# teshnizi/GraphEnvs

Hardware: AMD Instinct MI355X
Metric: env-steps/sec (whole node), ShortestPath-v0 n=64 m=192 batch=65536, 1/2/4/8 GPU (higher is better)
Workload: dtype u64; 1 GPU; ShortestPath-v0 n_nodes=64 n_edges=192 weighted, 65536 env slots per GPU, random valid actions on device, same-step autoreset (seed-exact G(n,m)+features on device); envs_per_gpu=65536, prefetch_period=0, episodes_finished_per_gpu=6165512, settle_steps=128, parallelism=batch shard x1, no collective

## Files before the change

graphenvs_amd/csrc/ge_api.hip:

```cpp
#include <math.h>
#include <stdio.h>
#include <stdlib.h>
#include <string.h>

#include <initializer_list>
#include <memory>
#include <new>
#include <vector>

#include "ge_params.h"
#include "ge_platform.h"
#include "ge_reset.h"
#include "ge_features.h"
#include "ge_step.h"
#include "ge_tsp_eval.h"
#include "ge_spare.h"
#include "ge_policy.h"

#define GE_MAX_BUCKETS 4
struct GeBucket {
  bool used;
  bool list_only;
  struct { int lds, pre, grid; } graph;
  struct { int lds, pre_off, threads, grid; } gen;
};
struct GePlan {
  int n_buckets;
  GeBucket bk[GE_MAX_BUCKETS];
  int nseed;
  int nseed2;
  bool feat_fast;
  int f64_lds, f64_pre_off, feat_grid;
  GeLds inject;
  int pol_group, pol_grid;
};
static int bucket_of(int n) { return n <= 128 ? 0 : (n <= 256 ? 1 : (n <= 512 ? 2 : 3)); }
static bool takes_generic(const GeParams &C) { return C.n > 64 || C.spatial; }

typedef void (*GeBaselineFn)(GeParams, GeRagged, int, uint8_t *, uint64_t);
struct GeKernels {
  void (*reset)(GeParams, GeRagged, const uint32_t *, GeRun, GeInject, int, int);
  void (*features)(GeParams, GeRagged, GeRun, int, int);
  void (*features64)(GeParams, GeRagged, GeRun, int);
  void (*feat_combine)(GeParams, GeRagged, GeRun);
  void (*swap)(GeParams, GeRagged, GeRagged, ge_buffers, int);
  void (*sample)(GeParams, GeRagged, uint64_t, int64_t *);
  void (*policy_head[GE_POL_MODES])(GeParams, GeRagged, GePolicyIO);
  void (*policy_grad)(GeParams, GeRagged, GePolicyIO);
  void (*dc_range)(GeParams, GeRagged, const int64_t *);
  void (*tsp_closure)(GeParams, GeRagged, int, uint8_t *, uint64_t, int);
  GeBaselineFn tsp_tour, mis_baseline, steiner_baseline;
  void (*step[2])(GeParams, GeRagged, const int64_t *, uint64_t);
  int step_threads;
  size_t step_lds;
  bool step_quad;
  void (*step_path64[2][2])(GeParams, const int64_t *, uint64_t);
};

struct ge_engine {
  GeParams P;
  ge_config cfg;
  GeKernels k = {};
  GePlan plan = {};
  hipEvent_t ev[4];
  bool have_events = false;
  int n_classes = 0;
  GeRagged R = {};
  int aw_max;
  std::vector<GeParams> classes;
  bool loaded = false;
  bool seeded = false;
  bool streams = false;
  bool spares = false;
  GeParams PS;
  GeRagged RS = {};
  std::vector<GeParams> classesS;
  int period = 0, swap_parts = 1;
  int64_t pending_calls = 0;
  int32_t *refill_list = nullptr, *refill_count = nullptr;
};

static GeRun run_full() { GeRun r = {GE_ITEMS_ALL, 1, 0, 0, 0, 0, 0}; return r; }
static GeRun run_inject(bool seeds) { GeRun r = {GE_ITEMS_ALL, seeds ? 2 : 0, 0, 0, 1, 0, 0}; return r; }
static GeRun run_continue() { GeRun r = {GE_ITEMS_ALL, 0, 1, 1, 0, 0, 0}; return r; }
static GeRun run_queue(const ge_engine *e) { GeRun r = {GE_ITEMS_QUEUE, 0, 1, 0, 0, 0, e->spares ? 2 : GE_SEED_DEPTH, e->plan.nseed2}; return r; }
static GeRun run_refill() { GeRun r = {GE_ITEMS_QUEUE, 0, 1, 0, 0, 1, 2}; return r; }
static GeRun as_list(GeRun r) { r.items = GE_ITEMS_LIST; return r; }


static thread_local char g_err[256] = "";
static int fail(int code, const char *msg) { snprintf(g_err, sizeof(g_err), "%s", msg); return code; }
extern "C" const char *ge_last_error(void) { return g_err; }
extern "C" int ge_abi_version(void) { return GE_ABI_VERSION; }
#ifndef GE_SOURCE_HASH
#define GE_SOURCE_HASH "unknown"
#endif
static const char g_source_hash[] = "GE_SOURCE_HASH=" GE_SOURCE_HASH;
extern "C" const char *ge_source_hash(void) { return g_source_hash + 15; }

static const int kMaxLds = 160 * 1024;
static const GeInject kNoInject = {nullptr, nullptr, nullptr, nullptr, nullptr};
static int step_blocks(int64_t B) { return (int)((B + GE_STEP_BLOCK - 1) / GE_STEP_BLOCK); }
static int prefix_bytes(int64_t B) { return (step_blocks(B) + 2) * 4; }
static bool carves_fit(std::initializer_list<int> bytes) { for (int b : bytes) if (b > kMaxLds) return false; return true; }
static int resident_grid(int lds, int64_t B) {
  int per_cu = kMaxLds / (lds > 0 ? lds : 1);
  if (per_cu > 16) per_cu = 16;
  if (per_cu < 1) per_cu = 1;
// ... 128 lines not shown
  if (P.feat_parts > 1 && !bufs->feat_scratch) return fail(GE_E_BADARG, "feat_scratch required (ge_layout.feat_parts > 1)");
  if (P.spatial && !bufs->sw64) return fail(GE_E_BADARG, "spatial TSP needs sw64");
  if (eval_slot_bytes(P) && !bufs->eval_scratch) return fail(GE_E_BADARG, "is_eval_env of TSP / unweighted MaxIndependentSet / SteinerTree (1 < n_dests < n - 1) needs eval_scratch (ge_layout.eval_scratch_bytes)");
  if (P.W == 1 && !bufs->node_rec) return fail(GE_E_BADARG, "n_nodes <= 64 needs node_rec");
  if (prunes(P) && P.W > GE_MAXW && !bufs->prune_scratch)
    return fail(GE_E_BADARG, "parenting >= 2 on more than 512 nodes needs prune_scratch ([B, 4, W] uint64)");
  return GE_OK;
}

static bool edge_quad(const ge_engine *e) {
  static const bool off = getenv("GE_NO_EDGE_QUAD") != nullptr;
  return !off && (e->P.env_type == GE_STEINER_TREE || e->P.env_type == GE_MULTICAST_ROUTING) && ge_edge_fits(e->aw_max, e->P.W);
}

static bool path64(const ge_engine *e) {
  return e->n_classes == 0 && (e->P.env_type == GE_SHORTEST_PATH || e->P.env_type == GE_LONGEST_PATH) && e->P.W == 1 && e->P.parenting < 2;
}

template <int ENV, bool RAGGED>
static void select_kernels(ge_engine *e) {
  GeKernels &k = e->k;
  k.reset = ge_k_reset<ENV, RAGGED>;
  k.features = ge_k_features<RAGGED>;
  k.features64 = ge_k_features64<RAGGED>;
  k.feat_combine = ge_k_feat_combine<RAGGED>;
  k.swap = ge_k_swap<RAGGED>;
  k.sample = ge_k_sample<RAGGED>;
  k.policy_head[GE_POL_SAMPLE] = ge_k_policy_head<RAGGED, GE_POL_SAMPLE>;
  k.policy_head[GE_POL_GREEDY] = ge_k_policy_head<RAGGED, GE_POL_GREEDY>;
  k.policy_head[GE_POL_EVALUATE] = ge_k_policy_head<RAGGED, GE_POL_EVALUATE>;
  k.policy_grad = ge_k_policy_grad<RAGGED>;
  k.dc_range = ge_k_dc_range<RAGGED>;
  k.tsp_closure = ge_k_tsp_closure<RAGGED>;
  k.tsp_tour = ge_k_tsp_tour<RAGGED>;
  k.mis_baseline = ge_k_mis_baseline<RAGGED>;
  k.steiner_baseline = ge_k_steiner_baseline<RAGGED>;
  k.step[0] = ge_k_step<ENV, false, RAGGED, 0>; k.step[1] = ge_k_step<ENV, true, RAGGED, 0>;
  k.step_threads = GE_STEP_BLOCK;
  k.step_lds = (size_t)GE_STEP_BLOCK * e->P.W * 8 + GE_STEP_BLOCK + 64;
  if constexpr (ENV == GE_STEINER_TREE || ENV == GE_MULTICAST_ROUTING) {
    if (edge_quad(e)) {
      k.step[0] = ge_k_step_edge<ENV, false, RAGGED>; k.step[1] = ge_k_step_edge<ENV, true, RAGGED>;
      k.step_quad = true;
      k.step_threads = GE_EDGE_THREADS;
      k.step_lds = ge_edge_lds_bytes(e->aw_max, e->P.W) + (RAGGED ? GE_EDGE_CLASS_BYTES : 0);
    }
  }
// ... 42 lines not shown
    if (gen > gen_body) gen_body = gen;
    K.graph.grid = resident_grid(graph, P.B);
    K.graph.pre = P.lds.pre; K.graph.lds = graph;
    if (rg && P.lds.pre != 0) K.graph.lds = behind(graph, K.graph.pre);
    if (K.graph.lds > graph_lds) graph_lds = K.graph.lds;
    K.gen.threads = GE_WAVE * waves;
    K.gen.pre_off = P.ldsf.pre; K.gen.lds = P.ldsf.total;
    if (rg) K.gen.lds = behind(K.list_only ? all : gen, K.gen.pre_off);
    K.gen.grid = resident_grid(K.gen.lds, P.B);
    if (K.list_only && (rg || K.gen.grid > 8)) K.gen.grid = 8;
    if (K.gen.lds > gen_lds) gen_lds = K.gen.lds;
  }
  if (!rg) L.inject = inject_carve(P, P.B);
  if (!carves_fit({graph_lds, L.inject.total, gen_lds})) return fail(GE_E_TOOBIG, "per-env graph does not fit 160 KiB of LDS");
  L.nseed = (resident_grid(graph_lds, P.B) + 63) / 64;
  if (!raise_lds((const void *)e->k.reset, graph_lds > L.inject.total ? graph_lds : L.inject.total)) return fail(GE_E_LAUNCH, "cannot raise the dynamic LDS limit of the reset kernel");
  if (!raise_lds((const void *)e->k.step[0], e->k.step_lds) || !raise_lds((const void *)e->k.step[1], e->k.step_lds))
    return fail(GE_E_LAUNCH, e->k.step_quad ? "cannot raise the dynamic LDS limit of the edge step kernel" : "cannot raise the dynamic LDS limit of the step kernel");
  L.f64_pre_off = ge_align16(f64_body);
  L.f64_lds = L.feat_fast ? L.f64_pre_off + GE_F64_ITEMS * 4 * 4 + 16 : 0;
  L.nseed2 = (GE_SEED_SPLIT && !rg && L.feat_fast) ? (L.nseed * GE_WAVE + GE_SEED2_ITEMS - 1) / GE_SEED2_ITEMS : 0;
  const int seed2_lds = GE_SEED2_WAVES * GE_SEED2_WAVE_BYTES;
  if (L.nseed2 > 0 && L.f64_lds < seed2_lds) L.f64_lds = seed2_lds;
  if (!carves_fit({L.f64_lds})) return fail(GE_E_TOOBIG, "feature kernel does not fit LDS");
  if (!raise_lds((const void *)e->k.features, gen_lds)) return fail(GE_E_LAUNCH, "cannot raise the dynamic LDS limit of the feature kernel");
  if (L.feat_fast && !raise_lds((const void *)e->k.features64, L.f64_lds)) return fail(GE_E_LAUNCH, "cannot raise the dynamic LDS limit of the n<=64 feature kernel");
  L.feat_grid = resident_grid(L.feat_fast ? L.f64_lds : gen_body, P.B);
  int a_max = 0;
  for (const GeParams *C = first; C < first + n_classes; C++) if (C->A > a_max) a_max = C->A;
  L.pol_group = 4;
  while (L.pol_group < 64 && L.pol_group < a_max) L.pol_group <<= 1;
  const int64_t waves = ((int64_t)P.B * L.pol_group + GE_WAVE - 1) / GE_WAVE;
  L.pol_grid = (int)((waves + GE_POL_THREADS / GE_WAVE - 1) / (GE_POL_THREADS / GE_WAVE));
  return GE_OK;
}

extern "C" int ge_create(const ge_config *cfg, const ge_buffers *bufs, ge_engine **out) {
  if (!bufs || !out) return fail(GE_E_BADARG, "null argument");
  GeParams P;
  int rc = derive(cfg, P);
  if (rc != GE_OK) return rc;
  rc = check_buffers(P, bufs);
  if (rc != GE_OK) return rc;
  P.buf = *bufs;
  std::unique_ptr<ge_engine> e(new (std::nothrow) ge_engine());
  if (!e) return fail(GE_E_BADARG, "out of host memory");
  e->P = P; e->cfg = *cfg; e->aw_max = P.AW;
  rc = finish_create(e.get());
  if (rc == GE_OK) *out = e.release();
// ... 111 lines not shown
  int rc = GE_OK;
  if (e->n_classes == 0) rc = check_image(e->P, sp[0].image);
  for (int c = 0; c < e->n_classes && rc == GE_OK; c++) rc = check_image(e->classes[c], sp[c].image);
  if (rc != GE_OK) return rc;
  e->refill_list = sp[0].refill_list; e->refill_count = sp[0].refill_count;
  e->PS = image_view(e->P, sp[0].image, e->refill_list, e->refill_count);
  if (e->n_classes > 0) {
    e->classesS.resize(e->n_classes);
    for (int c = 0; c < e->n_classes; c++) e->classesS[c] = image_view(e->classes[c], sp[c].image, e->refill_list, e->refill_count);
    if (hipMemcpy(class_table_spare, e->classesS.data(), sizeof(GeParams) * (size_t)e->n_classes, hipMemcpyHostToDevice) != hipSuccess)
      return fail(GE_E_LAUNCH, "cannot copy the spare class table to the device");
    e->RS = e->R; e->RS.classes = (const GeParams *)class_table_spare;
  }
  e->P.spare_state = sp[0].state; e->P.swap_list = sp[0].swap_list; e->P.swap_count = sp[0].swap_count;
  e->PS.spare_state = sp[0].state;
  e->period = sp[0].period; e->pending_calls = 0;
  const GeParams &P = e->P;
  const int64_t slot_bytes = (int64_t)P.n * P.F * 4 + (int64_t)P.E * (16 + 4 * P.Fe + 2 + 1 + (P.buf.rev_edge ? 4 : 0)) + (int64_t)P.n * P.W * 8 * (P.buf.range_bits ? 2 : 1) + P.A;
  int parts = (int)(slot_bytes / 8192); if (parts < 1) parts = 1; if (parts > 16) parts = 16;
  if (parts >= 4) parts = GE_SWAP_GROUPS;
  e->swap_parts = parts;
  e->spares = true;
  e->plan.nseed2 = 0;
  return GE_OK;
}

extern "C" int ge_destroy(ge_engine *e) {
  if (!e) return GE_OK;
  if (e->have_events) for (int k = 0; k < 4; k++) (void)hipEventDestroy(e->ev[k]);
  delete e;
  return GE_OK;
}

static int check_launch(const char *what) {
  static const bool debug_sync = getenv("GE_DEBUG_SYNC") != nullptr;
  if (debug_sync) {
    fprintf(stderr, "[graphenvs] %s ...\n", what); fflush(stderr);
    const hipError_t hs = hipDeviceSynchronize();
    fprintf(stderr, "[graphenvs] %s %s\n", what, hs == hipSuccess ? "done" : hipGetErrorString(hs)); fflush(stderr);
    if (hs != hipSuccess) { snprintf(g_err, sizeof(g_err), "%s: %s (GE_DEBUG_SYNC)", what, hipGetErrorString(hs)); return GE_E_LAUNCH; }
  }
  hipError_t hr = hipGetLastError();
  if (hr != hipSuccess) { snprintf(g_err, sizeof(g_err), "%s: %s", what, hipGetErrorString(hr)); return GE_E_LAUNCH; }
  return GE_OK;
}

// ... 18 lines not shown
  const int g = spread(e->plan.feat_grid, B, queue);
  return small && g > 64 ? 64 : g;
}

static int generic_grid(const ge_engine *e, const GeBucket &K, const GeParams &V, GeRun run, bool small) {
  const bool queue = run.items == GE_ITEMS_QUEUE, list = e->plan.feat_fast;
  if (K.list_only) return K.gen.grid;
  int64_t want = list ? (int64_t)K.gen.grid * (queue ? 1 : 4) : fast_grid(e, V.B, queue, small);
  want *= ge_feat_workgroups(V.feat_parts);
  if (!list && queue && !run.refill && want > 4608) want = 4608;
  if (small && want > 288) want = 288;
  return want > 65535 * 16 ? 65535 * 16 : (int)want;
}

static int launch_features(ge_engine *e, const GeParams &V, const GeRagged &VR, GeRun run, bool small, void *stream) {
  const GePlan &L = e->plan;
  const GeRun rest = L.feat_fast ? as_list(run) : run;
  int rc = GE_OK;
  if (L.feat_fast) {
    const bool queue = run.items == GE_ITEMS_QUEUE;
    const int nseed2 = queue ? run.seed_split : 0;
    int grid = fast_grid(e, V.B, queue, small) - nseed2;
    if (grid < 1) grid = 1;
    GE_LAUNCH(e->k.features64, grid + nseed2, GE_F64_THREADS, L.f64_lds, stream, V, VR, run, L.f64_pre_off);
    rc = check_launch("feature kernel (n <= 64)");
  }
  for (int b = 0; b < L.n_buckets && rc == GE_OK; b++) {
    const GeBucket &K = L.bk[b];
    if (!K.used) continue;
    GE_LAUNCH(e->k.features, generic_grid(e, K, V, run, small), K.gen.threads, K.gen.lds, stream, V, VR, rest, K.gen.pre_off, e->n_classes > 0 ? b : -1);
    rc = check_launch(L.feat_fast ? "feature kernel (fallback list)" : "feature kernel");
  }
  if (rc != GE_OK || V.feat_parts == 1) return rc;
  return launch_combine(e, V, VR, rest, small, stream);
}

static int launch_seq_baseline(ge_engine *e, const GeParams &P, const GeRagged &VR, int queue, void *stream) {
  const uint64_t slot_bytes = e->n_classes > 0 ? 0 : eval_slot_bytes(P);
  const int pre = prefix_bytes(P.B);
  int g = (P.B + GE_TSP_EVAL_THREADS - 1) / GE_TSP_EVAL_THREADS; if (g > 4096) g = 4096;
  if (P.env_type == GE_MAX_INDEPENDENT_SET) {
    GE_LAUNCH(e->k.mis_baseline, g, GE_TSP_EVAL_THREADS, pre, stream, P, VR, queue, (uint8_t *)P.buf.eval_scratch, slot_bytes);
    return check_launch("MaxIndependentSet baseline kernel");
  }
  if (P.env_type == GE_STEINER_TREE) {
    GE_LAUNCH(e->k.steiner_baseline, g, GE_TSP_EVAL_THREADS, pre, stream, P, VR, queue, (uint8_t *)P.buf.eval_scratch, slot_bytes);
    return check_launch("SteinerTree baseline kernel");
// ... 351 lines not shown
```

graphenvs_amd/csrc/ge_features.h:

```cpp
#pragma once
#include "ge_params.h"
#include "ge_platform.h"
#include "ge_reset.h"

struct GeFctx {
  uint64_t *abits; int *rowptr; uint16_t *scw;
  uint64_t *quads; uint32_t *rq; int zq;
  uint8_t *c8;
  double *sigma, *delta, *coeff, *bcw;
  double *bcw0; int wave_f64;
  double *bc, *clos;
  double *prx, *prn, *sinv, *diff, *diff2, *clus;
  uint8_t *mark;
  uint16_t *ord, *lvl;
};

GE_DEV GeFctx ge_carve_f(const GeParams &P, int tid) {
  unsigned char *s = ge_dyn_smem();
  const GeLdsF &L = P.ldsf;
  const int n = P.n, an = ((n * 8 + 15) & ~15) / 8;
  GeFctx c;
  c.rowptr = (int *)(s + L.rowptr); c.quads = (uint64_t *)(s + L.colw); c.c8 = (uint8_t *)(s + L.colw); c.rq = (uint32_t *)(s + L.rq); c.zq = L.zq;
  c.bc = (double *)(s + L.bc); c.clos = (double *)(s + L.clos);
  unsigned char *w = s + L.wave0 + (tid >> 6) * L.wave_stride;
// ... 640 lines not shown
  for (int64_t g = (int64_t)ge_bid() * ge_bdim() + ge_tid(); g < (int64_t)count * nmax; g += (int64_t)ge_gdim() * ge_bdim()) {
    const int item = (int)(g / nmax), v = (int)(g % nmax);
    int env = queue ? ge_queue_slot(P, pre, item) : (list ? P.buf.work_list[item] : item);
    int cls = 0;
    if constexpr (RAGGED) { cls = R.slot_class[env]; env -= R.class_start[cls]; }
    const GeParams &C = RAGGED ? R.classes[cls] : P;
    const int n = C.n, nparts = C.feat_parts;
    if (v >= n || nparts == 1) continue;
    double acc = 0.0;
    for (int p = 0; p < nparts; p++) acc += C.buf.feat_scratch[((int64_t)env * nparts + p) * n + v];
    if (n > 2) acc *= 1.0 / (double)((int64_t)(n - 1) * (int64_t)(n - 2));
    C.buf.x[((int64_t)env * n + v) * C.F + C.nflag + 1] = (float)acc;
  }
}

#ifndef GE_F64_WPS
#define GE_F64_WPS 6
#endif
#if GE_F64_WPS > 0
#define GE_F64_KERNEL GE_KERNEL_LB(GE_F64_THREADS, GE_F64_WPS)
#else
#define GE_F64_KERNEL GE_KERNEL
#endif
template <bool RAGGED>
GE_F64_KERNEL ge_k_features64(GeParams P, GeRagged R, GeRun run, int tail_off) {
  const int nblk = (P.B + GE_STEP_BLOCK - 1) / GE_STEP_BLOCK;
  int *const pre = (int *)ge_dyn_smem();
  int *const items = (int *)(ge_dyn_smem() + tail_off);
  int *const ovf_flag = items + GE_F64_ITEMS * 4;
  const bool queue = run.items == GE_ITEMS_QUEUE;
  const int nseed2 = (GE_SEED_SPLIT && queue) ? run.seed_split : 0;
  if (nseed2 > 0 && ge_bid() < nseed2) {
    ge_wave_priority(GE_PRIO_SEED2);
    for (int g0 = ge_bid() * GE_SEED2_ITEMS;; g0 += nseed2 * GE_SEED2_ITEMS) {
      const int tid = ge_tid_fresh();
      if (tid < GE_WAVE) ge_queue_prefix_wave(P, pre, tid);
      ge_sync();
      const int count = pre[nblk];
      if (g0 >= count) break;
      const int q = g0 + tid;
      uint32_t sb = 0xffffffffu;
      if (tid < GE_SEED2_ITEMS && q < count) {
        const int env = ge_queue_slot(P, pre, q);
        sb = (uint32_t)env * GE_SEED_DEPTH + (uint32_t)((P.buf.episode[env] + run.seed_ahead) % GE_SEED_DEPTH);
        ge_advance_episode(P, env);
      }
      ge_sync();
      if (tid < GE_SEED2_ITEMS) ge_seed_pass2_group(P, ge_dyn_smem(), sb, tid);
      ge_sync();
    }
    return;
  }
  const int bid = ge_bid() - nseed2, gdim = ge_gdim() - nseed2;
  int count = P.B;
  for (int base = 0;; base += GE_F64_ITEMS) {
    const int tid = ge_tid_fresh();
    if (queue) {
      if (tid < GE_WAVE) ge_queue_prefix_wave(P, pre, tid);
      ge_sync();
      count = pre[nblk];
    }
    const int total = count + (count + 3) / 4;
    if (bid + (int64_t)base * gdim >= total) break;
    if (tid < GE_F64_ITEMS * 4) {
      const int64_t q = bid + (int64_t)(base + (tid >> 2)) * gdim;
      const int sub = tid & 3;
      int qi = -1;
      if (q < count) qi = sub == 0 ? (int)q : -1;
      else if (q < total) { const int64_t k = 4 * (q - count) + sub; qi = k < count ? (int)k : -1; }
      items[tid] = qi < 0 ? -1 : (queue ? ge_queue_slot(P, pre, qi) : qi);
    }
    ge_sync();
    for (int i = 0; i < GE_F64_ITEMS; i++) {
      const int64_t q = bid + (int64_t)(base + i) * gdim;
      if (q >= total) break;
      if (q < count) {
        const int env = items[4 * i];
        if (queue && nseed2 == 0 && ge_tid() == 0) ge_finish_item(P, run, env);
        if constexpr (RAGGED) {
          const int cls = ge_slot_class(R, env);
          const GeParams &C = R.classes[cls];
          if (C.n > 64) {
            if (ge_tid() == 0) { int k = atomicAdd(&P.buf.work_count[0], 1); P.buf.work_list[k] = env; }
            continue;
          }
          ge_f64_walk_env(C, env - R.class_start[cls], ovf_flag, P.buf.work_count, P.buf.work_list, env);
        } else {
          ge_f64_walk_env(P, env, ovf_flag, P.buf.work_count, P.buf.work_list, env);
        }
      } else {
        const int t2 = ge_tid_fresh();
        const int wv = t2 >> 6, lane = t2 & (GE_WAVE - 1);
        const int env = items[4 * i + wv];
        if (env >= 0) {
          if constexpr (RAGGED) {
            const int cls = ge_slot_class(R, env);
            const GeParams &C = R.classes[cls];
            if (C.n <= 64) ge_f64_node_env(C, env - R.class_start[cls], ge_dyn_smem() + wv * ge_f64_node_wave_bytes(R.f64_tsp_e, C.env_type == GE_TSP), lane);
          } else {
// ... 10 lines not shown
```

graphenvs_amd/csrc/ge_params.h:

```cpp
#pragma once
#include <stdint.h>

#include "../../include/graphenvs.h"

#define GE_WAVE 64
#define GE_MT_N 624
#define GE_MT_M 397
#ifndef GE_DC_LANES
#define GE_DC_LANES 16
#endif
#ifndef GE_STEP_BLOCK
#define GE_STEP_BLOCK 256
#endif
#define GE_RESET_THREADS 128
#define GE_SEED_TILE_STRIDE 68
#define GE_SEED_LDS_BYTES (2 * 16 * GE_SEED_TILE_STRIDE * 4 + 64 * 4 + 64)
#ifndef GE_SEED_SPLIT
#define GE_SEED_SPLIT 1
#endif
#define GE_SEED2_WAVE_BYTES (16 * GE_SEED_TILE_STRIDE * 4 + 64 * 4)
#ifndef GE_SEED2_WAVES
#define GE_SEED2_WAVES 4
#endif
#define GE_SEED2_ITEMS (GE_SEED2_WAVES * 64)
// ... 48 lines not shown
  double n_choices;
  double max_distance;
  double dt_min, dt_max;
  int64_t env_index_base, seed_stride, node_id_base, edge_row_stride;
  ge_buffers buf;
  GeLds lds;
  GeLdsF ldsf;
  uint8_t *spare_state;
  int32_t *swap_list, *swap_count;
  int32_t bucket;
  int64_t policy_off;
};

enum { GE_ITEMS_ALL = 0, GE_ITEMS_QUEUE = 1, GE_ITEMS_LIST = 2 };
struct GeRun {
  int32_t items;
  int32_t restart;
  int32_t next;
  int32_t cont;
  int32_t inject;
  int32_t refill;
  int32_t seed_ahead;
  int32_t seed_split;
};

struct GeRagged {
  const GeParams *classes;
  const int32_t *slot_class;
  const int32_t *class_start;
  int32_t n_classes;
  int32_t f64_tsp_e;
};

static inline int ge_align16(int v) { return (v + 15) & ~15; }

static inline void ge_make_lds(GeParams &P, int queue_B) {
  GeLds &L = P.lds;
  int o = 0;
  auto take = [&](int bytes) { int r = o; o = ge_align16(o + bytes); return r; };
  L.mt = take(GE_MT_N * 4);
  L.mt2 = take(GE_MT_N * 4);
  {
    const bool matrix_env = P.env_type == GE_SHORTEST_PATH || P.env_type == GE_LONGEST_PATH || P.env_type == GE_STEINER_TREE ||
                            P.env_type == GE_MULTICAST_ROUTING || P.env_type == GE_DISTRIBUTION_CENTER || P.env_type == GE_PERISHABLE_DELIVERY;
    const int matrix = (P.np_early && matrix_env && P.weighted) ? ((P.n * P.n + 7) / 8) * 4 : 0;
    int nb = matrix > 16 ? matrix : 16; if (P.m > nb) nb = P.m; if (P.n > nb) nb = P.n;
// ... 96 lines not shown
```

graphenvs_amd/csrc/ge_reset.h:

```cpp
#pragma once
#include "ge_params.h"
#include "ge_platform.h"

GE_DEV double ge_wlut(int code) {
  const int k = (code >= 3 && code <= 9) ? code : 10;
  return (double)k / 10.0;
}

GE_DEV uint32_t ge_temper(uint32_t y) {
  y ^= (y >> 11);
  y ^= (y << 7) & 0x9d2c5680u;
  y ^= (y << 15) & 0xefc60000u;
  y ^= (y >> 18);
  return y;
}

GE_DEV void ge_mt_twist(uint32_t *mt, int lane) {
  const int lo[3] = {0, GE_MT_N - GE_MT_M, 2 * (GE_MT_N - GE_MT_M)}, hi[3] = {GE_MT_N - GE_MT_M, 2 * (GE_MT_N - GE_MT_M), GE_MT_N};
#pragma unroll
  for (int ph = 0; ph < 3; ph++) {
    uint32_t a[4], b[4], c[4];
#pragma unroll
    for (int k = 0; k < 4; k++) {
      const int i = lo[ph] + lane + 64 * k;
// ... 1119 lines not shown
      for (int k0 = rowptr[u]; k0 < r1; k0 += 4) {
        uint32_t e[4]; double sv[4];
#pragma unroll
        for (int j = 0; j < 4; j++) e[j] = (uint32_t)colw[k0 + j < r1 ? k0 + j : k0];
#pragma unroll
        for (int j = 0; j < 4; j++) sv[j] = S[(int)(e[j] >> 4) * ss];
#pragma unroll
        for (int j = 0; j < 4; j++) {
          const int v = (int)(e[j] >> 4);
          const double d = du + ge_wlut((int)(e[j] & 15u));
          if (k0 + j < r1 && d <= cutoff && d < sv[j]) {
            S[v * ss] = d; reached |= 1ull << v;
            if (d + 0.3 <= cutoff) nxt |= 1ull << v;
          }
        }
      }
    }
    cur = nxt;
  }
  return reached;
}

template <int ENV>
GE_DEV void ge_write_edge_slabs(const GeParams &P, const GeRctx &c, int env, int tid, int nthreads) {
  constexpr int t = ENV;
  const ge_buffers &G = P.buf;
  const int n = P.n, W = P.W, E = P.E;
  const int64_t nbase = (int64_t)env * n, ebase = (int64_t)env * E, Ne = P.edge_row_stride;
  for (int idx = tid; idx < E; idx += nthreads) {
    int u = ge_row_of(P, c, idx), v = ge_list_nbr(P, c, idx), code = ge_list_code(P, c, idx);
    G.edge_index[ebase + idx] = P.node_id_base + nbase + u;
    G.edge_index[Ne + ebase + idx] = P.node_id_base + nbase + v;
    float wv = (t == GE_DENSEST_SUBGRAPH || t == GE_MAX_INDEPENDENT_SET) ? 1.f : (float)ge_wlut(code);
    if (P.spatial) wv = (float)G.sw64[ebase + ge_sorted_pos_p(P, c, u, v)];
    if (P.Fe == 2) { G.edge_attr[(ebase + idx) * 2] = wv; G.edge_attr[(ebase + idx) * 2 + 1] = 0.f; }
    else G.edge_attr[ebase + idx] = wv;
    G.colw[ebase + idx] = (uint16_t)((v << 4) | code);
    G.scode[ebase + idx] = P.nowsort ? (uint8_t)code : c.wsort[idx];
    if (G.rev_edge) {
      const int r0 = c.rowptr[v], r1 = c.rowptr[v + 1];
      int r = -1;
      for (int k0 = r0; k0 < r1 && r < 0; k0 += 4) {
        int w[4];
#pragma unroll
        for (int j = 0; j < 4; j++) w[j] = (int)(c.colw[k0 + j < r1 ? k0 + j : r0] >> 4);
#pragma unroll
        for (int j = 3; j >= 0; j--) if (k0 + j < r1 && w[j] == u) r = k0 + j;
      }
      G.rev_edge[ebase + idx] = r;
    }
  }
  for (int v = tid; v <= n; v += nthreads) G.row_ptr[(int64_t)env * (n + 1) + v] = c.rowptr[v];
  for (int i = tid; i < n * W; i += nthreads) G.adj_bits[nbase * W + i] = c.abits[i];
  if (G.node_rec) {
    for (int v = tid; v < n; v += nthreads) {
      uint64_t codes = 0; int d = c.rowptr[v + 1] - c.rowptr[v]; if (d > 16) d = 16;
      for (int k = 0; k < d; k++) codes |= (uint64_t)(c.wsort[c.rowptr[v] + k] & 15) << (4 * k);
      G.node_rec[(nbase + v) * 2] = c.abits[v]; G.node_rec[(nbase + v) * 2 + 1] = codes;
    }
  }
}

template <int ENV>
GE_DEV void ge_reset_env(const GeParams &P, int env, const uint32_t *seeds, const GeRun &run, const GeInject &inj) {
  const int tid = ge_tid_fresh();
  const int lane = tid & (GE_WAVE - 1);
  const int wv = tid >> 6;
  const int n = P.n, ng = P.ng, W = P.W, m = P.m, E = P.E, F = P.F, T = P.T;
  constexpr int t = ENV;
  const bool path_like_t = (t == GE_SHORTEST_PATH || t == GE_LONGEST_PATH || t == GE_STEINER_TREE || t == GE_MULTICAST_ROUTING);
  GeRctx c = ge_carve(P);
  const int64_t nbase = (int64_t)env * n, ebase = (int64_t)env * E;
  const bool restart = run.restart != 0;
  const bool next = run.next != 0;
  const bool queued = run.items == GE_ITEMS_QUEUE && !run.refill;
  const int64_t episode = restart ? 0 : P.buf.episode[env] + (next ? 1 : 0);
  const uint32_t seed = restart ? (run.restart == 1 ? seeds[env] : inj.seeds[env]) : P.buf.seed[env] + (next ? (uint32_t)P.seed_stride : 0u);
  const int ring = (int)(episode % GE_SEED_DEPTH);
  auto keep_at = [&](int which) -> uint32_t * { return P.buf.stream_state ? P.buf.stream_state + ((int64_t)env * 2 + which) * GE_STREAM_WORDS : nullptr; };
  auto pos0 = [&](int which) -> int { return run.cont ? (int)keep_at(which)[GE_MT_N] : GE_MT_N; };
  const uint32_t *mt_src = P.buf.mt_state + ((int64_t)env * GE_SEED_DEPTH + ring) * 2 * GE_MT_N;
  if (run.cont) mt_src = keep_at(0);
  int src = 0, dest = -1;
  int ppd_pk[5] = {-1, -1, -1, -1, -1}, ppd_dp[5] = {-1, -1, -1, -1, -1};
  bool gen_failed = false;
  double ppd_dt = 0.0;
  if (wv == 1) {
    if (!run.inject) { ge_numpy_wave<ENV>(P, c, run.cont ? keep_at(1) : mt_src + GE_MT_N, lane, env, pos0(1), keep_at(1)); ge_sync(); }
    ge_sync();
    ge_write_edge_slabs<ENV>(P, c, env, tid, 2 * GE_WAVE);
    ge_sync();
    return;
  }

  GE_STAMP(0);
  if (!run.inject) {
    ge_mt_load(c.mt, mt_src, lane);
    GE_STAMP(1);
    int pypos = pos0(0);
    int ppd_attempt = 0, ppd_pos = 0;
    bool failed = false;
    const int shift = 32 - (32 - ge_clz32((uint32_t)ng));
    for (;;) {
      GE_STAMP(29);
      for (int i = lane; i < n * W; i += GE_WAVE) c.abits[i] = 0ull;
      ge_wave_sync();
      if (P.complete) {
        for (int v = lane; v < ng; v += GE_WAVE)
          for (int w = 0; w < W; w++) {
            int lo = w * 64, hi = lo + 64; if (hi > ng) hi = ng;
            uint64_t bitsw = (hi <= lo) ? 0ull : ((hi - lo == 64) ? ~0ull : ((1ull << (hi - lo)) - 1ull));
            if ((v >> 6) == w) bitsw &= ~(1ull << (v & 63));
            c.abits[v * W + w] = bitsw;
          }
// ... 117 lines not shown
            c.abits[u * W + (v >> 6)] |= 1ull << (v & 63); c.abits[v * W + (u >> 6)] |= 1ull << (u & 63);
            c.elist[cnt++] = (uint32_t)u | ((uint32_t)v << 16);
          }
      }
      ge_wave_sync();
      if (t == GE_PERISHABLE_DELIVERY) { if (ppd_attempt == 0) { ge_sync(); ppd_pos = c.misc[2]; } for (int i = 0; i < P.n_dests; i++) { ppd_pk[i] = i; ppd_dp[i] = P.n_dests + i; } }
    }
    if (P.buf.stream_state) {
      ge_mt_save(keep_at(0), c.mt, pypos, lane);
      if (t == GE_PERISHABLE_DELIVERY) ge_mt_save(keep_at(1), c.mt2, ppd_pos, lane);
    }
  } else {
    for (int i = lane; i < n * W; i += GE_WAVE) c.abits[i] = 0ull;
    for (int v = lane; v < n; v += GE_WAVE) c.fill[v] = 0;
    ge_wave_sync();
    for (int idx = lane; idx < E; idx += GE_WAVE) {
      int u = (int)inj.links[(ebase + idx) * 2], v = (int)inj.links[(ebase + idx) * 2 + 1];
      atomicAdd(&c.fill[u], 1);
      atomicOr((unsigned long long *)&c.abits[u * W + (v >> 6)], (unsigned long long)(1ull << (v & 63)));
    }
    ge_wave_sync();
  }

  GE_STAMP(2);
  if (!run.inject) {
    for (int v = lane; v < n; v += GE_WAVE) { int d = 0; for (int w = 0; w < W; w++) d += ge_popc64(c.abits[v * W + w]); c.fill[v] = d; }
    ge_wave_sync();
  }
  {
    int carry = 0;
    for (int k0 = 0; k0 < n; k0 += GE_WAVE) {
      int v = k0 + lane; int d = v < n ? c.fill[v] : 0;
      int incl = ge_wave_incl_scan(d, lane);
      if (v < n) c.rowptr[v] = carry + incl - d;
      carry += ge_shfl_i32(incl, GE_WAVE - 1);
    }
    if (lane == 0) c.rowptr[n] = carry;
    ge_wave_sync();
  }
  if (run.inject) {
    for (int idx = lane; idx < E; idx += GE_WAVE) {
      int u = (int)inj.links[(ebase + idx) * 2], v = (int)inj.links[(ebase + idx) * 2 + 1];
      c.colw[idx] = (uint16_t)((v << 4) | (inj.wcode[ebase + idx] & 15));
      if (!P.complete) c.tmp[idx] = (uint32_t)u;
    }
    ge_wave_sync();
  } else if (P.complete) {
// ... 8 lines not shown
    ge_wave_sync();
    for (int id = lane; id < m; id += GE_WAVE) {
      uint32_t e = c.elist[id]; int u = (int)(e & 0xffffu), v = (int)(e >> 16);
      int s = c.rowptr[u] + atomicAdd(&c.fill[u], 1); c.tmp[s] = ((uint32_t)id << 16) | (uint32_t)v;
      int s2 = c.rowptr[v] + atomicAdd(&c.fill[v], 1); c.tmp[s2] = ((uint32_t)id << 16) | (uint32_t)u;
    }
    ge_wave_sync();
    for (int v = lane; v < n; v += GE_WAVE) {
      int lo = c.rowptr[v], hi = c.rowptr[v + 1];
      for (int a = lo + 1; a < hi; a++) {
        uint32_t key = c.tmp[a]; int b = a - 1;
        while (b >= lo && c.tmp[b] > key) { c.tmp[b + 1] = c.tmp[b]; b--; }
        c.tmp[b + 1] = key;
      }
    }
    ge_wave_sync();
    for (int idx = lane; idx < E; idx += GE_WAVE) c.colw[idx] = (uint16_t)(((c.tmp[idx] & 0xffffu) << 4) | 10u);
    ge_wave_sync();
    for (int v = lane; v < n; v += GE_WAVE) for (int k = c.rowptr[v]; k < c.rowptr[v + 1]; k++) c.tmp[k] = (uint32_t)v;
    ge_wave_sync();
  }

  GE_STAMP(3);
  if (!run.inject && t != GE_PERISHABLE_DELIVERY) ge_sync();
  if (!run.inject) {
    if (!P.nowsort) for (int idx = lane; idx < E; idx += GE_WAVE) c.wsort[idx] = 10;
    ge_wave_sync();
    const bool path_like = path_like_t;
    const bool matrix_w = path_like_t || t == GE_DISTRIBUTION_CENTER || t == GE_PERISHABLE_DELIVERY;
    if (P.weighted && matrix_w && P.np_early) {
      for (int idx = lane; idx < E; idx += GE_WAVE) {
        int u = ge_row_of(P, c, idx), v = c.colw[idx] >> 4;
        int a = u < v ? u : v, b = u < v ? v : u, cell = a * n + b;
        c.wsort[ge_sorted_pos_p(P, c, u, v)] = (uint8_t)((c.wm[cell >> 3] >> (4 * (cell & 7))) & 15u);
      }
    } else if (P.spatial) {
      const double *xy = (const double *)(c.wm + 4 * n);
      for (int idx = lane; idx < E; idx += GE_WAVE) {
        int u = ge_row_of(P, c, idx), v = c.colw[idx] >> 4;
        int a = u < v ? u : v, b = u < v ? v : u;
        double dx = xy[2 * a] - xy[2 * b], dy = xy[2 * a + 1] - xy[2 * b + 1];
        P.buf.sw64[ebase + ge_sorted_pos_p(P, c, u, v)] = __builtin_sqrt(dx * dx + dy * dy);
      }
    } else if (P.weighted && t == GE_TSP && P.complete) {
      if (!P.nowsort) for (int idx = lane; idx < E; idx += GE_WAVE) {
        const int u = ge_row_of(P, c, idx), v = ge_list_nbr(P, c, idx);
        const int a = u < v ? u : v, b = u < v ? v : u;
// ... 121 lines not shown
    const int nf = P.nflag;
    for (int idx = lane; idx < n * nf; idx += GE_WAVE) {
      int v = idx / nf, col = idx % nf; float val = 0.f;
      bool is_t = (tbits[v >> 6] >> (v & 63)) & 1ull;
      if (t == GE_SHORTEST_PATH || t == GE_STEINER_TREE) val = (col == 0) ? (v == src ? 1.f : 0.f) : (is_t ? 1.f : 0.f);
      else if (t == GE_LONGEST_PATH) val = (col == 0) ? (v == src ? 1.f : 0.f) : (is_t ? 1.f : ((P.parenting == 0 && v == src) ? 2.f : 0.f));
      else if (t == GE_TSP) val = (col == 1 && v == 0) ? 1.f : ((P.spatial && col >= 2) ? (float)((const double *)(c.wm + 4 * n))[2 * v + (col - 2)] : 0.f);
      else if (t == GE_MAX_INDEPENDENT_SET) val = (col == 0) ? (float)ge_wlut(c.fill[v]) : 0.f;
      else if (t == GE_MULTICAST_ROUTING)
        val = (col == 0) ? (v == src ? 1.f : 0.f) : (col == 1) ? (is_t ? 1.f : 0.f) : (col == 2) ? (float)max_distance : (v == src ? 0.f : -1.f);
      else if (t == GE_PERISHABLE_DELIVERY) {
        const int pi = (col - 1) % 5;
        if (col == 0) val = (v == 0) ? 1.f : 0.f;
        else if (pi >= P.n_dests) val = 0.f;
        else if (col <= 5) val = (v == c.perm[pi]) ? 1.f : 0.f;
        else if (col <= 10) val = (v == c.perm[P.n_dests + pi]) ? 1.f : 0.f;
        else val = (float)ppd_dt;
      }
      else if (t == GE_DISTRIBUTION_CENTER)
        val = (col == 0) ? (float)((const uint8_t *)c.wm)[P.cost_off + v] : (col == 2) ? (is_t ? 1.f : 0.f) : (col == 4) ? (float)P.max_distance : 0.f;
      G.x[(nbase + v) * F + col] = val;
    }
  }
  ge_write_edge_slabs<ENV>(P, c, env, tid, 2 * GE_WAVE);
  const int A = P.A, AW = P.AW;
  const bool node_started = path_like_t;
  uint64_t *prune = c.bits + 4 * W;
  if (lane < W) prune[lane] = ~0ull;
  ge_wave_sync();
  if (t == GE_LONGEST_PATH && P.parenting >= 2) {
    uint64_t *rem = c.bits + 5 * W;
    if (lane < W) rem[lane] = ((src >> 6) == lane) ? (1ull << (src & 63)) : 0ull;
    ge_wave_sync();
    ge_reach_wave(c, n, W, dest, rem, lane);
    if (lane < W) {
      uint64_t keep = c.bits[W + lane] & ~rem[lane];
      if (P.parenting == 3 && n - 1 <= n / 3) keep = ~rem[lane];
      prune[lane] = keep;
    }
    ge_wave_sync();
  } else if (t == GE_TSP && P.parenting >= 2) {
    uint64_t *rem = c.bits + 5 * W;
    for (int v = 1; v < n; v++) {
      if (!((c.abits[0 * W + (v >> 6)] >> (v & 63)) & 1ull)) continue;
      if (n - 2 == 0) break;
      if (lane < W) rem[lane] = (lane == 0 ? 1ull : 0ull) | (((v >> 6) == lane) ? (1ull << (v & 63)) : 0ull);
      ge_wave_sync();
// ... 64 lines not shown
  for (int idx = lane; idx < A; idx += GE_WAVE) G.mask[(int64_t)env * A + idx] = (uint8_t)((((uint64_t *)c.sigma)[idx >> 6] >> (idx & 63)) & 1ull);
  for (int w = lane; w < W; w += GE_WAVE) {
    uint64_t nb = 0;
    if (node_started && (src >> 6) == w) nb = 1ull << (src & 63);
    G.node_bits[(int64_t)env * W + w] = nb;
    G.target_bits[(int64_t)env * W + w] = tbits[w];
    if (G.cover_bits) G.cover_bits[(int64_t)env * W + w] = 0ull;
  }
  if (G.node_aux) {
    for (int v = lane; v < n; v += GE_WAVE) G.node_aux[nbase + v] = -1;
    ge_wave_sync();
    for (int k = c.rowptr[src] + lane; k < c.rowptr[src + 1]; k += GE_WAVE) G.node_aux[nbase + (c.colw[k] >> 4)] = k;
  }
  for (int k = lane; k < T; k += GE_WAVE) G.terminals[(int64_t)env * T + k] = (t == GE_TSP) ? 0 : ((t == GE_DENSEST_SUBGRAPH || t == GE_MAX_INDEPENDENT_SET) ? -1 : ((t == GE_DISTRIBUTION_CENTER && k >= P.n_dests) ? -1 : c.perm[k]));
  if (lane == 0) {
    const uint64_t head16 = (t == GE_DENSEST_SUBGRAPH || t == GE_MAX_INDEPENDENT_SET || t == GE_DISTRIBUTION_CENTER) ? GE_REC_HEAD_MASK : (uint64_t)src;
    uint64_t status = (queued && P.autoreset == 2) ? 3ull : 0ull;
    if (gen_failed) status = 4ull;
    const uint64_t aux = ((t == GE_SHORTEST_PATH || t == GE_LONGEST_PATH) && W == 1) ? (uint64_t)dest : 0ull;
    const uint64_t tstep = queued ? (G.slot_rec[2 * (int64_t)env + 1] >> GE_REC_TSTEP_SHIFT) : 0ull;
    G.slot_rec[2 * (int64_t)env] = 0ull;
    G.slot_rec[2 * (int64_t)env + 1] = head16 | (status << GE_REC_STATUS_SHIFT) | (aux << GE_REC_AUX_SHIFT) | (tstep << GE_REC_TSTEP_SHIFT);
    G.counters[env * 2] = 0; G.counters[env * 2 + 1] = 0;
    if (queued) G.final_heur[env] = G.heuristic[env];
    G.heuristic[env] = heuristic;
    if (run.items != GE_ITEMS_QUEUE) { G.seed[env] = seed; G.episode[env] = episode; }
    if (t == GE_PERISHABLE_DELIVERY && !run.inject) G.target_bits[(int64_t)env * W] = ge_f64_as_u64(ppd_dt);
  }
  ge_sync();
  GE_STAMP(10);
}

GE_DEV int ge_queue_prefix_of(const int32_t *rc, int nblk, int *pre, int lane) {
  int carry = 0;
  for (int k0 = 0; k0 < nblk; k0 += GE_WAVE) {
    int k = k0 + lane; int cnt = k < nblk ? rc[k] : 0;
    int incl = ge_wave_incl_scan(cnt, lane);
    if (k < nblk) pre[k] = carry + incl - cnt;
    carry += ge_shfl_i32(incl, GE_WAVE - 1);
  }
  if (lane == 0) pre[nblk] = carry;
  return carry;
}
GE_DEV int ge_queue_prefix_wave(const GeParams &P, int *pre, int lane) { return ge_queue_prefix_of(P.buf.reset_count, (P.B + GE_STEP_BLOCK - 1) / GE_STEP_BLOCK, pre, lane); }
GE_DEV int ge_queue_slot_of(const int32_t *list, int nblk, const int *pre, int q) {
  int lo = 0, hi = nblk;
  while (hi - lo > 1) { int mid = (lo + hi) >> 1; if (pre[mid] <= q) lo = mid; else hi = mid; }
  return list[lo * GE_STEP_BLOCK + (q - pre[lo])];
}
GE_DEV int ge_queue_slot(const GeParams &P, const int *pre, int q) { return ge_queue_slot_of(P.buf.reset_list, (P.B + GE_STEP_BLOCK - 1) / GE_STEP_BLOCK, pre, q); }



// ... 204 lines not shown
```

Before: 425.5 million env-steps/s.

## Split reset finish into parked records completed by the n<=64 feature kernel

Splits the reset kernel for shortest-path and MIS envs. Generation now parks the adjacency bits, terminals, edge list and weight codes in the edge_index buffer. The features64 kernel then unparks each record and runs the finish stage (degrees, weight sort, features, edge slabs, records) as extra work items dealt to blocks that have no walk item. The aim is to move the serial finish work off the reset critical path and balance it across idle feature blocks. The cost is an extra global write and read of the parked record, plus more complex work dealing.

```diff
diff --git a/graphenvs_amd/csrc/ge_api.hip b/graphenvs_amd/csrc/ge_api.hip
--- a/graphenvs_amd/csrc/ge_api.hip
+++ b/graphenvs_amd/csrc/ge_api.hip
@@ -29,6 +29,7 @@
   GeBucket bk[GE_MAX_BUCKETS];
   int nseed;
   int nseed2;
+  int finish_split;
   bool feat_fast;
   int f64_lds, f64_pre_off, feat_grid;
   GeLds inject;
@@ -42,6 +43,7 @@
   void (*reset)(GeParams, GeRagged, const uint32_t *, GeRun, GeInject, int, int);
   void (*features)(GeParams, GeRagged, GeRun, int, int);
   void (*features64)(GeParams, GeRagged, GeRun, int);
+  void (*features64_fin)(GeParams, GeRagged, GeRun, int);
   void (*feat_combine)(GeParams, GeRagged, GeRun);
   void (*swap)(GeParams, GeRagged, GeRagged, ge_buffers, int);
   void (*sample)(GeParams, GeRagged, uint64_t, int64_t *);
@@ -83,7 +85,7 @@
 static GeRun run_full() { GeRun r = {GE_ITEMS_ALL, 1, 0, 0, 0, 0, 0}; return r; }
 static GeRun run_inject(bool seeds) { GeRun r = {GE_ITEMS_ALL, seeds ? 2 : 0, 0, 0, 1, 0, 0}; return r; }
 static GeRun run_continue() { GeRun r = {GE_ITEMS_ALL, 0, 1, 1, 0, 0, 0}; return r; }
-static GeRun run_queue(const ge_engine *e) { GeRun r = {GE_ITEMS_QUEUE, 0, 1, 0, 0, 0, e->spares ? 2 : GE_SEED_DEPTH, e->plan.nseed2}; return r; }
+static GeRun run_queue(const ge_engine *e) { GeRun r = {GE_ITEMS_QUEUE, 0, 1, 0, 0, 0, e->spares ? 2 : GE_SEED_DEPTH, e->plan.nseed2, e->plan.finish_split}; return r; }
 static GeRun run_refill() { GeRun r = {GE_ITEMS_QUEUE, 0, 1, 0, 0, 1, 2}; return r; }
 static GeRun as_list(GeRun r) { r.items = GE_ITEMS_LIST; return r; }
 
@@ -258,7 +260,9 @@
   GeKernels &k = e->k;
   k.reset = ge_k_reset<ENV, RAGGED>;
   k.features = ge_k_features<RAGGED>;
-  k.features64 = ge_k_features64<RAGGED>;
+  k.features64 = ge_k_features64<RAGGED, -1>;
+  k.features64_fin = nullptr;
+  if constexpr (!RAGGED && ge_finish_splits<ENV>()) k.features64_fin = ge_k_features64<false, ENV>;
   k.feat_combine = ge_k_feat_combine<RAGGED>;
   k.swap = ge_k_swap<RAGGED>;
   k.sample = ge_k_sample<RAGGED>;
@@ -347,9 +351,12 @@
   L.nseed2 = (GE_SEED_SPLIT && !rg && L.feat_fast) ? (L.nseed * GE_WAVE + GE_SEED2_ITEMS - 1) / GE_SEED2_ITEMS : 0;
   const int seed2_lds = GE_SEED2_WAVES * GE_SEED2_WAVE_BYTES;
   if (L.nseed2 > 0 && L.f64_lds < seed2_lds) L.f64_lds = seed2_lds;
+  L.finish_split = (e->k.features64_fin && !rg && L.feat_fast && !P.complete && (!P.weighted || P.np_early) && eval_slot_bytes(P) == 0 &&
+                    P.lds.total <= L.f64_pre_off && ge_finish_rec_fits(P)) ? 1 : 0;
   if (!carves_fit({L.f64_lds})) return fail(GE_E_TOOBIG, "feature kernel does not fit LDS");
   if (!raise_lds((const void *)e->k.features, gen_lds)) return fail(GE_E_LAUNCH, "cannot raise the dynamic LDS limit of the feature kernel");
   if (L.feat_fast && !raise_lds((const void *)e->k.features64, L.f64_lds)) return fail(GE_E_LAUNCH, "cannot raise the dynamic LDS limit of the n<=64 feature kernel");
+  if (L.finish_split && !raise_lds((const void *)e->k.features64_fin, L.f64_lds)) return fail(GE_E_LAUNCH, "cannot raise the dynamic LDS limit of the n<=64 feature kernel (finish items)");
   L.feat_grid = resident_grid(L.feat_fast ? L.f64_lds : gen_body, P.B);
   int a_max = 0;
   for (const GeParams *C = first; C < first + n_classes; C++) if (C->A > a_max) a_max = C->A;
@@ -507,6 +514,7 @@
   e->swap_parts = parts;
   e->spares = true;
   e->plan.nseed2 = 0;
+  e->plan.finish_split = 0;
   return GE_OK;
 }
 
@@ -571,7 +579,8 @@
     const int nseed2 = queue ? run.seed_split : 0;
     int grid = fast_grid(e, V.B, queue, small) - nseed2;
     if (grid < 1) grid = 1;
-    GE_LAUNCH(e->k.features64, grid + nseed2, GE_F64_THREADS, L.f64_lds, stream, V, VR, run, L.f64_pre_off);
+    void (*const kernel)(GeParams, GeRagged, GeRun, int) = run.finish_split ? e->k.features64_fin : e->k.features64;
+    GE_LAUNCH(kernel, grid + nseed2, GE_F64_THREADS, L.f64_lds, stream, V, VR, run, L.f64_pre_off);
     rc = check_launch("feature kernel (n <= 64)");
   }
   for (int b = 0; b < L.n_buckets && rc == GE_OK; b++) {
diff --git a/graphenvs_amd/csrc/ge_features.h b/graphenvs_amd/csrc/ge_features.h
--- a/graphenvs_amd/csrc/ge_features.h
+++ b/graphenvs_amd/csrc/ge_features.h
@@ -686,7 +686,47 @@
 #else
 #define GE_F64_KERNEL GE_KERNEL
 #endif
-template <bool RAGGED>
+#ifndef GE_F64_FIN_CAP
+#define GE_F64_FIN_CAP 2
+#endif
+enum { GE_F64_NONE = 0, GE_F64_WALK = 1, GE_F64_NODE = 2, GE_F64_FINISH = 3 };
+struct GeF64Item { int kind, idx; };
+template <bool FIN>
+GE_DEV GeF64Item ge_f64_deal(int bid, int gdim, int k, int count) {
+  const int nodes = (count + 3) / 4;
+  GeF64Item none = {GE_F64_NONE, 0};
+  if (!FIN) {
+    const int64_t q = bid + (int64_t)k * gdim;
+    if (q < count) return GeF64Item{GE_F64_WALK, (int)q};
+    if (q < count + nodes) return GeF64Item{GE_F64_NODE, (int)(q - count)};
+    return none;
+  }
+  const int nwalk = bid < count ? (count - bid + gdim - 1) / gdim : 0;
+  if (k < nwalk) return GeF64Item{GE_F64_WALK, bid + k * gdim};
+  k -= nwalk;
+  const int walkers = count < gdim ? count : gdim, free = gdim - walkers;
+  const int64_t extras = (int64_t)count + nodes, dealt = (int64_t)free * GE_F64_FIN_CAP;
+  int64_t j = -1;
+  if (bid >= walkers && k < GE_F64_FIN_CAP) j = (bid - walkers) + (int64_t)k * free;
+  else j = dealt + bid + (int64_t)(bid >= walkers ? k - GE_F64_FIN_CAP : k) * gdim;
+  if (j >= extras) return none;
+  if (j < count) return GeF64Item{GE_F64_FINISH, (int)j};
+  return GeF64Item{GE_F64_NODE, (int)(j - count)};
+}
+
+template <int FIN>
+GE_DEV void ge_f64_finish_env(const GeParams &P, const GeRun &run, int env) {
+  if constexpr (FIN >= 0) {
+    const int tid = ge_tid_fresh();
+    const GeRctx c = ge_carve(P);
+    const GeInject none = {nullptr, nullptr, nullptr, nullptr, nullptr};
+    GeFinishIn in = {false, true, 0u, 0, {0, 0, 0, 0, 0}, {0, 0, 0, 0, 0}, 0.0};
+    in.gen_failed = ge_finish_unpark<FIN>(P, c, env, tid, GE_F64_THREADS);
+    ge_reset_finish<FIN>(P, env, run, none, c, in, tid, GE_F64_THREADS, false);
+  }
+}
+
+template <bool RAGGED, int FIN>
 GE_F64_KERNEL ge_k_features64(GeParams P, GeRagged R, GeRun run, int tail_off) {
   const int nblk = (P.B + GE_STEP_BLOCK - 1) / GE_STEP_BLOCK;
   int *const pre = (int *)ge_dyn_smem();
@@ -716,6 +756,7 @@
     return;
   }
   const int bid = ge_bid() - nseed2, gdim = ge_gdim() - nseed2;
+  constexpr bool fin = FIN >= 0;
   int count = P.B;
   for (int base = 0;; base += GE_F64_ITEMS) {
     const int tid = ge_tid_fresh();
@@ -724,21 +765,22 @@
       ge_sync();
       count = pre[nblk];
     }
-    const int total = count + (count + 3) / 4;
-    if (bid + (int64_t)base * gdim >= total) break;
+    if (ge_f64_deal<fin>(bid, gdim, base, count).kind == GE_F64_NONE) break;
     if (tid < GE_F64_ITEMS * 4) {
-      const int64_t q = bid + (int64_t)(base + (tid >> 2)) * gdim;
+      const GeF64Item it = ge_f64_deal<fin>(bid, gdim, base + (tid >> 2), count);
       const int sub = tid & 3;
       int qi = -1;
-      if (q < count) qi = sub == 0 ? (int)q : -1;
-      else if (q < total) { const int64_t k = 4 * (q - count) + sub; qi = k < count ? (int)k : -1; }
+      if (it.kind == GE_F64_WALK || it.kind == GE_F64_FINISH) qi = sub == 0 ? it.idx : -1;
+      else if (it.kind == GE_F64_NODE) { const int64_t k = 4 * (int64_t)it.idx + sub; qi = k < count ? (int)k : -1; }
       items[tid] = qi < 0 ? -1 : (queue ? ge_queue_slot(P, pre, qi) : qi);
     }
     ge_sync();
     for (int i = 0; i < GE_F64_ITEMS; i++) {
-      const int64_t q = bid + (int64_t)(base + i) * gdim;
-      if (q >= total) break;
-      if (q < count) {
+      const int kind = ge_f64_deal<fin>(bid, gdim, base + i, count).kind;
+      if (kind == GE_F64_NONE) break;
+      if (kind == GE_F64_FINISH) {
+        ge_f64_finish_env<FIN>(P, run, items[4 * i]);
+      } else if (kind == GE_F64_WALK) {
         const int env = items[4 * i];
         if (queue && nseed2 == 0 && ge_tid() == 0) ge_finish_item(P, run, env);
         if constexpr (RAGGED) {
diff --git a/graphenvs_amd/csrc/ge_params.h b/graphenvs_amd/csrc/ge_params.h
--- a/graphenvs_amd/csrc/ge_params.h
+++ b/graphenvs_amd/csrc/ge_params.h
@@ -94,6 +94,7 @@
   int32_t refill;
   int32_t seed_ahead;
   int32_t seed_split;
+  int32_t finish_split;
 };
 
 struct GeRagged {
diff --git a/graphenvs_amd/csrc/ge_reset.h b/graphenvs_amd/csrc/ge_reset.h
--- a/graphenvs_amd/csrc/ge_reset.h
+++ b/graphenvs_amd/csrc/ge_reset.h
@@ -1165,7 +1165,7 @@
 }
 
 template <int ENV>
-GE_DEV void ge_write_edge_slabs(const GeParams &P, const GeRctx &c, int env, int tid, int nthreads) {
+GE_DEV void ge_write_edge_slabs(const GeParams &P, const GeRctx &c, int env, int tid, int nthreads, bool adj = true) {
   constexpr int t = ENV;
   const ge_buffers &G = P.buf;
   const int n = P.n, W = P.W, E = P.E;
@@ -1194,7 +1194,7 @@
     }
   }
   for (int v = tid; v <= n; v += nthreads) G.row_ptr[(int64_t)env * (n + 1) + v] = c.rowptr[v];
-  for (int i = tid; i < n * W; i += nthreads) G.adj_bits[nbase * W + i] = c.abits[i];
+  if (adj) for (int i = tid; i < n * W; i += nthreads) G.adj_bits[nbase * W + i] = c.abits[i];
   if (G.node_rec) {
     for (int v = tid; v < n; v += nthreads) {
       uint64_t codes = 0; int d = c.rowptr[v + 1] - c.rowptr[v]; if (d > 16) d = 16;
@@ -1202,6 +1202,83 @@
       G.node_rec[(nbase + v) * 2] = c.abits[v]; G.node_rec[(nbase + v) * 2 + 1] = codes;
     }
   }
+}
+
+#ifndef GE_FINISH_SPLIT
+#define GE_FINISH_SPLIT 1
+#endif
+template <int ENV>
+constexpr bool ge_finish_splits() { return GE_FINISH_SPLIT && (ENV == GE_SHORTEST_PATH || ENV == GE_MAX_INDEPENDENT_SET); }
+static inline int ge_finish_rec_words(const GeParams &P) {
+  const int terms = P.env_type == GE_SHORTEST_PATH ? P.T : 0;
+  const int codes = !P.weighted ? 0 : ((P.env_type == GE_SHORTEST_PATH ? P.m : P.n) + 3) / 4;
+  return 1 + terms + P.m + codes;
+}
+static inline bool ge_finish_rec_fits(const GeParams &P) { return ge_finish_rec_words(P) <= 2 * P.E; }
+
+struct GeFinishIn {
+  bool gen_failed;
+  bool parked;
+  uint32_t seed; int64_t episode;
+  int ppd_pk[5], ppd_dp[5]; double ppd_dt;
+};
+
+template <int ENV>
+GE_DEV void ge_reset_finish(const GeParams &P, int env, const GeRun &run, const GeInject &inj, const GeRctx &c, const GeFinishIn &in, int tid, int nthreads, bool join);
+
+template <int ENV>
+GE_DEV void ge_finish_park(const GeParams &P, const GeRctx &c, int env, int tid, int nthreads, bool gen_failed) {
+  const int n = P.n, W = P.W, m = P.m;
+  const int64_t nbase = (int64_t)env * n;
+  uint32_t *rec = (uint32_t *)(P.buf.edge_index + (int64_t)env * P.E);
+  for (int i = tid; i < n * W; i += nthreads) P.buf.adj_bits[nbase * W + i] = c.abits[i];
+  if (tid == 0) rec[0] = gen_failed ? 1u : 0u;
+  const int terms = ENV == GE_SHORTEST_PATH ? P.T : 0;
+  for (int k = tid; k < terms; k += nthreads) rec[1 + k] = (uint32_t)c.perm[k];
+  uint32_t *el = rec + 1 + terms, *codes = el + m;
+  for (int id = tid; id < m; id += nthreads) el[id] = c.elist[id];
+  if (!P.weighted) return;
+  if (ENV == GE_SHORTEST_PATH) {
+    for (int w = tid; w < (m + 3) / 4; w += nthreads) {
+      uint32_t word = 0u;
+      for (int k = 0; k < 4 && 4 * w + k < m; k++) {
+        const uint32_t e = c.elist[4 * w + k]; const int u = (int)(e & 0xffffu), v = (int)(e >> 16);
+        const int cell = (u < v ? u : v) * n + (u < v ? v : u);
+        word |= ((c.wm[cell >> 3] >> (4 * (cell & 7))) & 15u) << (8 * k);
+      }
+      codes[w] = word;
+    }
+  } else {
+    for (int w = tid; w < (n + 3) / 4; w += nthreads) codes[w] = c.wm[w];
+  }
+}
+
+template <int ENV>
+GE_DEV bool ge_finish_unpark(const GeParams &P, const GeRctx &c, int env, int tid, int nthreads) {
+  const int n = P.n, W = P.W, m = P.m;
+  const int64_t nbase = (int64_t)env * n;
+  const uint32_t *rec = (const uint32_t *)(P.buf.edge_index + (int64_t)env * P.E);
+  const bool gen_failed = rec[0] != 0u;
+  for (int i = tid; i < n * W; i += nthreads) c.abits[i] = P.buf.adj_bits[nbase * W + i];
+  const int terms = ENV == GE_SHORTEST_PATH ? P.T : 0;
+  for (int k = tid; k < terms; k += nthreads) c.perm[k] = (int)rec[1 + k];
+  const uint32_t *el = rec + 1 + terms, *codes = el + m;
+  for (int id = tid; id < m; id += nthreads) c.elist[id] = el[id];
+  if (P.weighted) {
+    if (ENV == GE_SHORTEST_PATH) {
+      for (int i = tid; i < (n * n + 7) / 8; i += nthreads) c.wm[i] = 0u;
+      ge_sync();
+      for (int id = tid; id < m; id += nthreads) {
+        const uint32_t e = el[id]; const int u = (int)(e & 0xffffu), v = (int)(e >> 16);
+        const int cell = (u < v ? u : v) * n + (u < v ? v : u);
+        atomicOr(&c.wm[cell >> 3], ((codes[id >> 2] >> (8 * (id & 3))) & 15u) << (4 * (cell & 7)));
+      }
+    } else {
+      for (int w = tid; w < (n + 3) / 4; w += nthreads) c.wm[w] = codes[w];
+    }
+  }
+  ge_sync();
+  return gen_failed;
 }
 
 template <int ENV>
@@ -1216,7 +1293,6 @@
   const int64_t nbase = (int64_t)env * n, ebase = (int64_t)env * E;
   const bool restart = run.restart != 0;
   const bool next = run.next != 0;
-  const bool queued = run.items == GE_ITEMS_QUEUE && !run.refill;
   const int64_t episode = restart ? 0 : P.buf.episode[env] + (next ? 1 : 0);
   const uint32_t seed = restart ? (run.restart == 1 ? seeds[env] : inj.seeds[env]) : P.buf.seed[env] + (next ? (uint32_t)P.seed_stride : 0u);
   const int ring = (int)(episode % GE_SEED_DEPTH);
@@ -1224,15 +1300,22 @@
   auto pos0 = [&](int which) -> int { return run.cont ? (int)keep_at(which)[GE_MT_N] : GE_MT_N; };
   const uint32_t *mt_src = P.buf.mt_state + ((int64_t)env * GE_SEED_DEPTH + ring) * 2 * GE_MT_N;
   if (run.cont) mt_src = keep_at(0);
-  int src = 0, dest = -1;
   int ppd_pk[5] = {-1, -1, -1, -1, -1}, ppd_dp[5] = {-1, -1, -1, -1, -1};
   bool gen_failed = false;
   double ppd_dt = 0.0;
+  const bool split = ge_finish_splits<ENV>() && run.finish_split != 0;
+  const bool join = !run.inject && t != GE_PERISHABLE_DELIVERY;
   if (wv == 1) {
-    if (!run.inject) { ge_numpy_wave<ENV>(P, c, run.cont ? keep_at(1) : mt_src + GE_MT_N, lane, env, pos0(1), keep_at(1)); ge_sync(); }
-    ge_sync();
-    ge_write_edge_slabs<ENV>(P, c, env, tid, 2 * GE_WAVE);
-    ge_sync();
+    if (!run.inject) ge_numpy_wave<ENV>(P, c, run.cont ? keep_at(1) : mt_src + GE_MT_N, lane, env, pos0(1), keep_at(1));
+    if (!run.inject && t == GE_PERISHABLE_DELIVERY) ge_sync();
+    if (split) {
+      ge_sync();
+      ge_finish_park<ENV>(P, c, env, tid, 2 * GE_WAVE, false);
+      ge_sync();
+    } else {
+      const GeFinishIn none = {false, false, seed, episode, {-1, -1, -1, -1, -1}, {-1, -1, -1, -1, -1}, 0.0};
+      ge_reset_finish<ENV>(P, env, run, inj, c, none, tid, 2 * GE_WAVE, join);
+    }
     return;
   }
 
@@ -1396,7 +1479,45 @@
     ge_wave_sync();
   }
 
-  GE_STAMP(2);
+  if (split) {
+    GE_STAMP(2);
+    ge_sync();
+    ge_finish_park<ENV>(P, c, env, tid, 2 * GE_WAVE, gen_failed);
+    ge_sync();
+    GE_STAMP(10);
+    return;
+  }
+  GeFinishIn fin = {gen_failed, false, seed, episode, {0, 0, 0, 0, 0}, {0, 0, 0, 0, 0}, ppd_dt};
+  if (t == GE_PERISHABLE_DELIVERY) for (int i = 0; i < 5; i++) { fin.ppd_pk[i] = ppd_pk[i]; fin.ppd_dp[i] = ppd_dp[i]; }
+  ge_reset_finish<ENV>(P, env, run, inj, c, fin, tid, 2 * GE_WAVE, join);
+}
+
+template <int ENV>
+GE_DEV void ge_reset_finish(const GeParams &P, int env, const GeRun &run, const GeInject &inj, const GeRctx &c, const GeFinishIn &in, int tid, int nthreads, bool join) {
+  const int lane = tid & (GE_WAVE - 1);
+  const int wv = tid >> 6;
+  const int n = P.n, ng = P.ng, W = P.W, m = P.m, E = P.E, F = P.F, T = P.T;
+  constexpr int t = ENV;
+  const bool path_like_t = (t == GE_SHORTEST_PATH || t == GE_LONGEST_PATH || t == GE_STEINER_TREE || t == GE_MULTICAST_ROUTING);
+  const int64_t nbase = (int64_t)env * n, ebase = (int64_t)env * E;
+  if (wv != 0) {
+    if (join) ge_sync();
+    ge_sync();
+    ge_write_edge_slabs<ENV>(P, c, env, tid, nthreads, !in.parked);
+    ge_sync();
+    return;
+  }
+  const bool queued = run.items == GE_ITEMS_QUEUE && !run.refill;
+  auto keep_at = [&](int which) -> uint32_t * { return P.buf.stream_state ? P.buf.stream_state + ((int64_t)env * 2 + which) * GE_STREAM_WORDS : nullptr; };
+  auto pos0 = [&](int which) -> int { return run.cont ? (int)keep_at(which)[GE_MT_N] : GE_MT_N; };
+  const bool gen_failed = in.gen_failed;
+  const uint32_t seed = in.seed; const int64_t episode = in.episode;
+  const int (&ppd_pk)[5] = in.ppd_pk, (&ppd_dp)[5] = in.ppd_dp;
+  const double ppd_dt = in.ppd_dt;
+  int src = 0, dest = -1;
+  (void)ng; (void)m;
+
+  if (!in.parked) GE_STAMP(2);
   if (!run.inject) {
     for (int v = lane; v < n; v += GE_WAVE) { int d = 0; for (int w = 0; w < W; w++) d += ge_popc64(c.abits[v * W + w]); c.fill[v] = d; }
     ge_wave_sync();
@@ -1451,7 +1572,7 @@
   }
 
   GE_STAMP(3);
-  if (!run.inject && t != GE_PERISHABLE_DELIVERY) ge_sync();
+  if (join) ge_sync();
   if (!run.inject) {
     if (!P.nowsort) for (int idx = lane; idx < E; idx += GE_WAVE) c.wsort[idx] = 10;
     ge_wave_sync();
@@ -1619,7 +1740,7 @@
       G.x[(nbase + v) * F + col] = val;
     }
   }
-  ge_write_edge_slabs<ENV>(P, c, env, tid, 2 * GE_WAVE);
+  ge_write_edge_slabs<ENV>(P, c, env, tid, nthreads, !in.parked);
   const int A = P.A, AW = P.AW;
   const bool node_started = path_like_t;
   uint64_t *prune = c.bits + 4 * W;
@@ -1730,13 +1851,18 @@
     G.slot_rec[2 * (int64_t)env] = 0ull;
     G.slot_rec[2 * (int64_t)env + 1] = head16 | (status << GE_REC_STATUS_SHIFT) | (aux << GE_REC_AUX_SHIFT) | (tstep << GE_REC_TSTEP_SHIFT);
     G.counters[env * 2] = 0; G.counters[env * 2 + 1] = 0;
-    if (queued) G.final_heur[env] = G.heuristic[env];
+#if defined(GE_STAMP_SLOTS) && !defined(GE_EMU)
+    if (queued && !in.parked)
+#else
+    if (queued)
+#endif
+      G.final_heur[env] = G.heuristic[env];
     G.heuristic[env] = heuristic;
     if (run.items != GE_ITEMS_QUEUE) { G.seed[env] = seed; G.episode[env] = episode; }
     if (t == GE_PERISHABLE_DELIVERY && !run.inject) G.target_bits[(int64_t)env * W] = ge_f64_as_u64(ppd_dt);
   }
   ge_sync();
-  GE_STAMP(10);
+  if (!in.parked) GE_STAMP(10);
 }
 
 GE_DEV int ge_queue_prefix_of(const int32_t *rc, int nblk, int *pre, int lane) {
```

Result: slower. 351.6 million env-steps/s (-17.4%).
